# TritonDataCenter/containerpilot

Hardware: NVIDIA H100
Metric: events/sec through Bus.Publish (deliveries/s = 32-byte records landed in subscriber mailboxes) (higher is better)
Workload: dtype u8

## Files before the change

containerpilot_b200/csrc/cpbus.cu:

```cuda
#include "cpbus_kernels.cuh"

#include <algorithm>
#include <chrono>
#include <cstdio>
#include <cstdlib>
#include <cstring>
#include <deque>
#include <mutex>
#include <new>
#include <string>
#include <thread>
#include <unordered_map>
#include <vector>

using namespace cpbus_dev;

namespace {

thread_local char g_cuda_err[256] = "";

#define CK(call)                                                                                   \
  do {                                                                                             \
    cudaError_t e_ = (call);                                                                       \
    if (e_ != cudaSuccess) {                                                                       \
// ... 250 lines not shown
  }
  cudaLaunchConfig_t cfg{};
  cfg.gridDim = dim3(grid); cfg.blockDim = dim3(kThreads); cfg.dynamicSmemBytes = smem; cfg.stream = b->stream;
  cudaLaunchAttribute attr[1];
  attr[0].id = cudaLaunchAttributeProgrammaticStreamSerialization;
  attr[0].val.programmaticStreamSerializationAllowed = 1;
  cfg.attrs = attr; cfg.numAttrs = b->pdl && kind != kLaunchRound ? 1 : 0;
  CK(cudaLaunchKernelEx(&cfg, kernel, p));
  CK(cudaGetLastError());
  return CPBUS_OK;
}

uint64_t max_window(const cpbus* b);

template <int ST>
int preload_round_fanouts() {
  void (*ks[])(FanoutParams) = {
      fanout_round_kernel<ST, false, false, false>, fanout_round_kernel<ST, false, true, false>,
      fanout_round_kernel<ST, true, false, false>, fanout_round_kernel<ST, true, true, false>,
      fanout_round_kernel<ST, false, false, true>, fanout_round_kernel<ST, false, true, true>,
      fanout_round_kernel<ST, true, false, false, true>, fanout_round_kernel<ST, true, true, false, true>};
  for (auto k : ks) CK(cudaFuncSetAttribute(k, cudaFuncAttributeMaxDynamicSharedMemorySize, kFanoutMaxSmem));
  return CPBUS_OK;
}

int preload_round_kernels(cpbus* b) {
  static bool done[64] = {};
  static std::mutex mu;
  std::lock_guard<std::mutex> g(mu);
  if (done[b->device & 63]) return CPBUS_OK;
  int rc;
  if ((rc = preload_round_fanouts<CPBUS_STORE_V4>()) || (rc = preload_round_fanouts<CPBUS_STORE_V8>()) ||
      (rc = preload_round_fanouts<CPBUS_STORE_BULK>()))
    return rc;
  cudaFuncAttributes a;
  CK(cudaFuncGetAttributes(&a, stream_round_decide_kernel));
  CK(cudaFuncGetAttributes(&a, stream_round_admit_kernel));
  CK(cudaFuncGetAttributes(&a, stream_round_agree_kernel));
  CK(cudaFuncGetAttributes(&a, consume_all_kernel));
  CK(cudaFuncGetAttributes(&a, digest_fold_kernel));
  done[b->device & 63] = true;
  return CPBUS_OK;
}

struct StreamArgs {
  const StreamHdr* hdr = nullptr; unsigned long long* ack = nullptr; unsigned long long seq = 0;
  const StreamHdr* next_hdr = nullptr;
  uint32_t off = 0; bool final = true;
  FollowRec* follow_rec = nullptr;
  bool follow_from_host = false;
  const RoundDev* round = nullptr;
};

int launch_fanout(cpbus* b, const cpbus_event* d_src, uint32_t n, uint64_t w, int staged = 0,
                  const cpbus_event* prefetch_src = nullptr, cpbus_event* prefetch_dst = nullptr, uint32_t prefetch_n = 0,
                  bool batch_dep = false, bool account = false, const StreamArgs* sa = nullptr) {
  if (b->n_next == 0 && !sa) return CPBUS_OK;
  if (n == 0 && b->n_timers == 0 && !sa) return CPBUS_OK;
  FanoutParams p{};
  p.batch = d_src; p.ring = b->d_ring; p.ctl = b->d_ctl; p.timers = b->d_timers; p.stats = b->d_stats; p.pow_table = b->d_pow; p.launch_seq = ++b->launch_seq;
  p.desc = b->d_desc + (p.launch_seq & 1) * ((fanout_desc_bytes(2048) + 255) & ~(size_t)255);
  p.desc_ready = b->d_desc_ready + (p.launch_seq & 1) * 16; p.w_now = w;
  p.result = b->d_result + (size_t)(p.launch_seq % kResultRing) * kResultSub;
  p.result_next = b->d_result + (size_t)((p.launch_seq + 1) % kResultRing) * kResultSub;
  p.batch_local = b->d_batch_local; p.staged = (uint32_t)staged;
  p.err_word = b->d_err; p.acct = account ? b->d_acct : nullptr;
  p.pf_state = b->d_pf_state; p.pf_buf = b->d_pf_buf; p.pf_stride = b->B; p.spin_us = b->stream_spin_us;
  if (sa) {
    p.stream_hdr = sa->hdr; p.stream_ack = sa->ack; p.stream_seq = sa->seq; p.stream_next_hdr = sa->next_hdr;
    p.stream_off = sa->off; p.stream_final = sa->final ? 1u : 0u;
  }
  const bool follow = sa && sa->follow_rec, round = sa && sa->round;
  const int kind = round ? kLaunchRound : follow ? kLaunchFollow : kLaunchPlain;
  p.round = round ? sa->round : nullptr;
  if (follow) {
    p.follow_clock = b->d_follow_clock; p.follow_rec = sa->follow_rec; p.follow_window = max_window(b);
    p.follow_from_host = sa->follow_from_host ? 1u : 0u;
  }
  p.prefetch_src = prefetch_src; p.prefetch_dst = prefetch_dst; p.prefetch_n = prefetch_n;
  p.batch_dep = batch_dep ? 1u : 0u; p.n_ev = n;
  p.n_subs = b->n_next; p.ring_cap = b->R; p.K = b->K; p.sub_base = b->cfg.sub_id_base;
  p.use_digest = b->use_digest; p.lossless = b->lossless; p.timers_on = b->n_timers > 0 && b->K > 0;
  p.smem_cap = (n + 31u) & ~31u;
  const size_t hot_bytes = (size_t)b->n_next * (sizeof(SubCtl) + (p.timers_on ? b->K * sizeof(DevTimer) : 0));
  p.hints = b->hints >= 0 ? (uint32_t)b->hints : (hot_bytes <= (64u << 20) ? 1u : 0u);
  const uint32_t need = (b->n_next + kWarpsPerCta - 1) / kWarpsPerCta;
  uint32_t grid = b->cfg.grid_ctas ? std::max(1u, std::min(b->cfg.grid_ctas, need)) : 0u;
  int rc;
  const bool pairs_on = b->n_paired > 0 && b->d_pairs;
  p.pairs = pairs_on ? b->d_pairs : nullptr;
  size_t smem = fanout_smem_bytes(p.smem_cap) + (pairs_on ? kPairFilterBytes : 0);
  if (!pairs_on && !p.timers_on && b->n_filtered > 0) {
    if (b->order_dirty) { const int rc_order = rebuild_order(b); if (rc_order) return rc_order; }
    if (b->n_order) {
      const uint32_t scale = std::max(1u, (p.n_ev + 128u) / 256u);
      uint32_t spw = b->subs_per_warp ? std::min(32u, b->subs_per_warp)
                                      : std::max(4u, std::min(16u / scale, b->n_order / (20480u * scale)));
      p.order = b->d_order; p.n_order = b->n_order; p.spw = spw;
      const uint32_t warps = (b->n_order + spw - 1) / spw;
      grid = std::max(1u, (warps + kWarpsPerCta - 1) / kWarpsPerCta);
    }
  }
  if (pairs_on && !b->cfg.grid_ctas) {
    const uint32_t blocks = (b->n_next + 31u) / 32u;
    grid = std::max(1u, std::min((blocks + kWarpsPerCta - 1) / kWarpsPerCta, (uint32_t)b->sm_count * 16u));
  }
  if (!pairs_on && !p.order) {
    uint32_t spw = b->subs_per_warp;
    if (grid) spw = std::max(1u, (need + grid - 1) / grid);
    else if (!spw) {
      const uint32_t scale = std::max(1u, (p.n_ev + 128u) / 256u);
      const uint32_t cap = std::max(1u, 16u / scale);
      spw = std::max(1u, std::min(cap, (need + (uint32_t)b->sm_count * 7 * scale) / ((uint32_t)b->sm_count * 14 * scale)));
    }
    p.spw = spw;
    grid = std::max(1u, (need + spw - 1) / spw);
    const size_t off = fanout_stage_off(p.smem_cap);
    const size_t per_sub = sizeof(SubCtl) + (p.timers_on ? (size_t)b->K * sizeof(DevTimer) : 0);
    const size_t min_round = (size_t)kWarpsPerCta * per_sub;
    const size_t ctas = std::max<size_t>(1, std::min<size_t>(kCtasPerSm, b->smem_per_sm / (off + min_round + b->smem_reserved)));
    const size_t room = std::min<size_t>(kFanoutMaxSmem, b->smem_per_sm / ctas - b->smem_reserved) - off;
    p.stage_subs = std::max<uint32_t>(kWarpsPerCta, (uint32_t)std::min<size_t>((size_t)kWarpsPerCta * spw, room / per_sub) & ~7u);
    smem = off + p.stage_subs * per_sub;
  }
  const int variant = pairs_on ? (p.use_digest ? 7 : 6) : (p.timers_on ? 2 : 0) | (p.use_digest ? 1 : 0) | (p.order ? 4 : 0);
#define CPBUS_DISPATCH(ST)                                                                \
  switch (variant) {                                                                     \
    case 0: rc = launch_fanout_t<ST, false, false, false>(b, p, grid, smem, kind); break;      \
    case 1: rc = launch_fanout_t<ST, false, true, false>(b, p, grid, smem, kind); break;       \
    case 2: rc = launch_fanout_t<ST, true, false, false>(b, p, grid, smem, kind); break;       \
    case 3: rc = launch_fanout_t<ST, true, true, false>(b, p, grid, smem, kind); break;        \
    case 4: rc = launch_fanout_t<ST, false, false, true>(b, p, grid, smem, kind); break;       \
    case 5: rc = launch_fanout_t<ST, false, true, true>(b, p, grid, smem, kind); break;        \
    case 6: rc = launch_fanout_t<ST, true, false, false, true>(b, p, grid, smem, kind); break; \
    default: rc = launch_fanout_t<ST, true, true, false, true>(b, p, grid, smem, kind); break; \
  }
  switch (b->store) {
    case CPBUS_STORE_V4: CPBUS_DISPATCH(CPBUS_STORE_V4); break;
    case CPBUS_STORE_BULK: CPBUS_DISPATCH(CPBUS_STORE_BULK); break;
    default: CPBUS_DISPATCH(CPBUS_STORE_V8); break;
  }
#undef CPBUS_DISPATCH
  if (rc) return rc;
  b->st.kernel_launches++;
  if (round) return CPBUS_OK;
  b->st.batches++;
  if (follow) return CPBUS_OK;
  b->last_watermark = w;
  if (account && n) dbg_mark_device_batch(b, p.launch_seq);
  return CPBUS_OK;
}

bool admit_fits(cpbus* b, uint32_t n, uint64_t w) {
  if (!b->lossless || b->n_next == 0) return true;
  const uint64_t need = admit_need(n, w, b->last_watermark, b->min_period, b->K, b->n_timers && b->K);
  if (b->room_lb >= need) { b->room_lb -= need; b->st.admit_skipped++; return true; }
  return false;
}

int admit_pass(cpbus* b, const cpbus_event* d_src, uint32_t n, uint64_t w, bool* ok, uint32_t* prefix) {
  CK(cudaMemsetAsync(&b->d_stats->admit_overflow, 0, 4 * sizeof(unsigned long long), b->stream));
  const uint32_t threads = 256, grid = (b->n_next + threads - 1) / threads;
  admit_kernel<<<grid, threads, 0, b->stream>>>(d_src, n, w, b->d_ctl, b->d_timers, b->n_next, b->R, b->K,
                                                b->cfg.sub_id_base, b->n_timers > 0 && b->K > 0, b->d_stats,
                                                b->n_paired > 0 ? b->d_pairs : nullptr);
  CK(cudaGetLastError());
  b->st.kernel_launches++; b->st.admit_passes++;
  CK(cudaMemcpyAsync(&b->h_stats->admit_overflow, &b->d_stats->admit_overflow, 4 * sizeof(unsigned long long),
// ... 1652 lines not shown
```

containerpilot_b200/csrc/cpbus_fanout_body.cuh:

```cuda
  constexpr bool STAGED = !ORDERED && !PAIRS;
  extern __shared__ __align__(128) unsigned char smem[];
  const uint32_t cap = p.smem_cap;
  cpbus_event* s_batch = reinterpret_cast<cpbus_event*>(smem);
  uint64_t* s_rhash = reinterpret_cast<uint64_t*>(smem + (size_t)cap * 32);
  uint2* s_meta = reinterpret_cast<uint2*>(smem + (size_t)cap * 40);
  uint64_t* s_q = reinterpret_cast<uint64_t*>(smem + (size_t)cap * 48);
  uint32_t* s_dsum = reinterpret_cast<uint32_t*>(s_q + cap + 2);
  uint32_t* s_present = s_dsum + 40;
  uint64_t* s_pow = s_q + cap + 2 + 20 + (PAIRS ? kPairFilterWords / 2 : 0);
  BatchSummary* s_sum = reinterpret_cast<BatchSummary*>(s_pow + cap + 66);
  uint32_t* s_tick = reinterpret_cast<uint32_t*>(s_sum + 1);
  const uint4* s_ctl4 = reinterpret_cast<const uint4*>(smem + fanout_stage_off(cap));
  const uint4* s_tim4 = s_ctl4 + 2u * p.stage_subs;

  const int tid = threadIdx.x, lane = tid & 31, warp = tid >> 5;
  uint32_t n = FOLLOW ? 0u : p.n_ev;
  uint64_t w_follow = 0;
  unsigned long long round_ack = 0;

  if (p.batch_dep) asm volatile("griddepcontrol.wait;" ::: "memory");
  const bool stream = p.staged == 2u;
  const uint32_t pf_slot = stream ? (uint32_t)(p.stream_seq % kStreamPrefetch) : 0u;
  uint32_t pos = ORDERED ? (blockIdx.x * kWarpsPerCta + warp) * p.spw : 0u;
  uint32_t my_ids = 0;
  if (ORDERED && pos + lane < min(pos + p.spw, p.n_order)) my_ids = __ldg(p.order + pos + lane);
  if (tid == 0) {
    mbar_init(&s_sum->mbar, 1); mbar_init(&s_sum->mbar_desc, 1); mbar_init(&s_sum->mbar_state, 1);
    s_sum->acc_deliv = 0; s_sum->acc_ticks = 0; s_sum->acc_dig_lo = 0; s_sum->acc_dig_hi = 0;
    s_sum->stream_local = (stream && !p.lossless && p.stream_off == 0 && __ldcg(p.pf_state + pf_slot) == p.stream_seq) ? 1u : 0u;
    s_sum->own_desc = blockIdx.x == 0 ? 1u : 0u; s_sum->abort_launch = 0;
  }
  __syncthreads();
  const bool stream_local = stream && s_sum->stream_local;
  const bool staged = FOLLOW || (p.staged && !stream_local);
  const cpbus_event* batch_src = stream_local ? p.pf_buf + (size_t)pf_slot * p.pf_stride : p.batch;
  if (tid == 0) {
    const uint32_t pow_bytes = ((cap + 65u) * 8u + 15u) & ~15u;
    const bool direct = n && !staged;
    mbar_expect_tx(&s_sum->mbar, (direct ? n * 32u : 0u) + pow_bytes);
    if (direct) bulk_g2s(s_batch, batch_src, n * 32u, &s_sum->mbar);
    bulk_g2s(s_pow, p.pow_table, pow_bytes, &s_sum->mbar);
  }

  const bool keep = p.hints & 1u;

  const uint32_t desc_bytes = 24u * cap + 16u + 160u + (PAIRS ? kPairFilterBytes : 0u);
  uint4* s_desc = reinterpret_cast<uint4*>(s_rhash);
  uint4* g_desc = reinterpret_cast<uint4*>(p.desc);
  constexpr unsigned long long kAbortBit = 1ull << 63;
  if (blockIdx.x != 0) {
    if (tid == 0) {
      unsigned long long seen = 0;
      if (!(p.hints & 2u)) {
        unsigned long long t0, t1;
        asm volatile("mov.u64 %0, %%globaltimer;" : "=l"(t0));
        const unsigned long long budget = stream ? 4000000000ull : 200000ull;
        do {
          asm volatile("ld.acquire.gpu.global.u64 %0, [%1];" : "=l"(seen) : "l"(p.desc_ready) : "memory");
          if ((seen & ~kAbortBit) >= p.launch_seq) break;
          asm volatile("mov.u64 %0, %%globaltimer;" : "=l"(t1));
        } while (t1 - t0 < budget);
      }
      if ((seen & ~kAbortBit) < p.launch_seq) s_sum->own_desc = 1u;
      else {
        const bool ab = (seen & kAbortBit) != 0;
        s_sum->abort_launch = ab ? 1u : 0u;
        asm volatile("fence.proxy.async;" ::: "memory");
        mbar_expect_tx(&s_sum->mbar_desc, desc_bytes);
        bulk_g2s(s_desc, g_desc, desc_bytes, &s_sum->mbar_desc);
        const uint32_t n_copy = FOLLOW ? (ab ? 0u : *reinterpret_cast<const volatile uint32_t*>(p.desc + 24u * cap + 16u + 4u * kFollowN)) : n;
        if (staged && n_copy && !ab) {
          mbar_wait(&s_sum->mbar, 0);
          mbar_expect_tx(&s_sum->mbar, n_copy * 32u);
          bulk_g2s(s_batch, p.batch_local, n_copy * 32u, &s_sum->mbar);
        }
      }
    }
    __syncthreads();
  }
  const bool own_desc = s_sum->own_desc != 0;
  const bool lead = blockIdx.x == 0;
  if (own_desc) {
    if (lead && tid < kResultSub * 4) reinterpret_cast<unsigned long long*>(p.result_next)[tid] = 0ull;
    if (tid < 40) s_dsum[tid] = 0;
    if constexpr (ROUND) {
      __syncthreads();
      if (tid == 0) {
        const volatile RoundDev* rd = p.round;
        if (!rd->go) s_sum->abort_launch = 1u;
        else {
          const unsigned long long w = rd->w;
          s_dsum[kFollowN] = rd->m; s_dsum[kFollowWLo] = (uint32_t)w; s_dsum[kFollowWHi] = (uint32_t)(w >> 32);
          s_dsum[kRoundSrc] = rd->src;
          if (lead && rd->final) round_ack = rd->q;
        }
      }
    } else if constexpr (FOLLOW) {
      __syncthreads();
      if (tid == 0) {
        unsigned long long seen = 0, t0, t1, tag = 0, prev = p.w_now, hw = 0;
        const unsigned long long budget = (p.spin_us ? (unsigned long long)p.spin_us : 2000000ull) * 1000ull;
        asm volatile("mov.u64 %0, %%globaltimer;" : "=l"(t0));
        unsigned int err = 0;
        uint32_t hn = 0;
        if (!p.follow_from_host) {
          const unsigned long long* pw = p.follow_clock + 2u * (uint32_t)((p.launch_seq - 1ull) & 1ull);
          for (;;) {
            asm volatile("ld.acquire.gpu.global.u64 %0, [%1];" : "=l"(tag) : "l"(pw + 1) : "memory");
            if (tag == p.launch_seq - 1ull) break;
            asm volatile("mov.u64 %0, %%globaltimer;" : "=l"(t1));
            if (t1 - t0 > budget) break;
            __nanosleep(64);
          }
          if (tag != p.launch_seq - 1ull) err = kErrStreamTimeout;
          else asm volatile("ld.relaxed.gpu.global.u64 %0, [%1];" : "=l"(prev) : "l"(pw) : "memory");
        }
        const bool skip = !err && prev == kFollowPoison;
        if (!err && !skip) {
          for (;;) {
            asm volatile("ld.acquire.sys.global.u64 %0, [%1];" : "=l"(seen) : "l"(&p.stream_hdr->seq) : "memory");
            if (seen >= p.stream_seq) break;
            asm volatile("mov.u64 %0, %%globaltimer;" : "=l"(t1));
            if (t1 - t0 > budget) break;
            __nanosleep(64);
          }
          if (seen != p.stream_seq) err = kErrStreamTimeout;
          else {
// ... 85 lines not shown
      const uint32_t lo = min(nd, (uint32_t)tid * E), hi = min(nd, lo + E);
      uint64_t sum = 0;
      for (uint32_t i = lo; i < hi; i++) sum += s_rhash[i] * s_pow[nd - 1 - i];
      uint64_t incl = sum;
#pragma unroll
      for (int o = 1; o < 32; o <<= 1) {
        const uint32_t l = __shfl_up_sync(0xffffffffu, (uint32_t)incl, o), h = __shfl_up_sync(0xffffffffu, (uint32_t)(incl >> 32), o);
        if (lane >= o) incl += ((uint64_t)h << 32) | l;
      }
      if (lane == 31) s_sum->red[warp] = incl;
      __syncthreads();
      uint64_t run = incl - sum;
      for (int w = 0; w < warp; w++) run += s_sum->red[w];
      for (uint32_t i = lo; i < hi; i++) { s_q[i] = run; run += s_rhash[i] * s_pow[nd - 1 - i]; }
      if (tid == 0) { uint64_t t = 0; for (int w = 0; w < kWarpsPerCta; w++) t += s_sum->red[w]; s_q[nd] = t; }
      __syncthreads();
    }
    if (PAIRS) {
      for (uint32_t i = tid; i < kPairFilterWords; i += kThreads) s_present[i] = 0u;
      __syncthreads();
      for (uint32_t i = tid; i < nd; i += kThreads) {
        if (s_meta[i].y != CPBUS_TARGET_ALL) continue;
        const uint32_t h = pair_key_hash(s_batch[i].code, s_batch[i].source_id);
        atomicOr(&s_present[(h & 32767u) >> 5], 1u << (h & 31u));
        atomicOr(&s_present[((h >> 15) & 32767u) >> 5], 1u << ((h >> 15) & 31u));
      }
      __syncthreads();
    }
    if (lead) {
      for (uint32_t i = tid; i < desc_bytes / 16u; i += kThreads) g_desc[i] = s_desc[i];
      __threadfence();
      __syncthreads();
      if (tid == 0) {
        const unsigned long long flag = p.launch_seq | (ab ? kAbortBit : 0ull);
        asm volatile("st.release.gpu.global.u64 [%0], %1;" ::"l"(p.desc_ready), "l"(flag) : "memory");
      }
    }
  } else {
    mbar_wait(&s_sum->mbar_desc, 0);
    if constexpr (FOLLOW) {
      n = s_sum->abort_launch ? 0u : s_dsum[kFollowN];
      w_follow = ((uint64_t)s_dsum[kFollowWHi] << 32) | s_dsum[kFollowWLo];
    }
    mbar_wait(&s_sum->mbar, (staged && n && !s_sum->abort_launch) ? 1u : 0u);
  }
  constexpr bool PLANAR = STORE != CPBUS_STORE_BULK && !ORDERED;
  const uint32_t hi_off = cap;
  if (PLANAR && n) {
    uint4* sq = reinterpret_cast<uint4*>(s_batch);
    uint4 v[8];
    __syncthreads();
#pragma unroll
    for (int r = 0; r < 8; r++) { const uint32_t q = tid + r * kThreads; if (q < 2u * n) v[r] = sq[q]; }
    __syncthreads();
#pragma unroll
    for (int r = 0; r < 8; r++) { const uint32_t q = tid + r * kThreads; if (q < 2u * n) sq[(q & 1u) * hi_off + (q >> 1)] = v[r]; }
    __syncthreads();
  }
  auto ev_ts = [&](uint32_t i) -> uint64_t {
    return PLANAR ? reinterpret_cast<const uint64_t*>(reinterpret_cast<const uint4*>(s_batch) + i)[1] : s_batch[i].ts_ns;
  };
  auto ev_code_src = [&](uint32_t i) -> uint2 {
    return PLANAR ? reinterpret_cast<const uint2*>(reinterpret_cast<const uint4*>(s_batch) + hi_off + i)[0] : make_uint2(s_batch[i].code, s_batch[i].source_id);
  };
  const bool aborted = s_sum->abort_launch != 0;
  const uint32_t K = p.K, J = K ? 32u / K : 32u;
  const uint32_t tk_slot = lane / J, tk_j = lane % J;
  const bool timers_on = TIMERS && p.timers_on && K;
  const uint32_t wstride = gridDim.x * kWarpsPerCta;
  uint32_t pos_end = (aborted || !ORDERED) ? 0u : min(pos + p.spw, p.n_order);
  const uint32_t pos_step = ORDERED ? 1u : kWarpsPerCta;
  const uint32_t pos0 = pos;
  uint32_t s = ORDERED ? __shfl_sync(0xffffffffu, my_ids, 0) : pos;
  if (!p.batch_dep) asm volatile("griddepcontrol.wait;" ::: "memory");
  asm volatile("griddepcontrol.launch_dependents;");
  const uint32_t rng_first = blockIdx.x * kWarpsPerCta * p.spw, rng_end = min(rng_first + kWarpsPerCta * p.spw, p.n_subs);
  auto stage_round = [&](uint32_t first) {
    if (!STAGED || tid != 0 || aborted || first >= rng_end) return;
    const uint32_t rn = min(p.stage_subs, rng_end - first);
    asm volatile("fence.proxy.async.shared::cta;" ::: "memory");
    const uint32_t tim_bytes = timers_on ? rn * K * (uint32_t)sizeof(DevTimer) : 0u;
    mbar_expect_tx(&s_sum->mbar_state, rn * (uint32_t)sizeof(SubCtl) + tim_bytes);
    bulk_g2s_hint(const_cast<uint4*>(s_ctl4), p.ctl + first, rn * (uint32_t)sizeof(SubCtl), &s_sum->mbar_state, keep);
    if (tim_bytes) bulk_g2s_hint(const_cast<uint4*>(s_tim4), p.timers + (size_t)first * K, tim_bytes, &s_sum->mbar_state, keep);
  };
  uint4 ca = make_uint4(0, 0, 0, 0), cb = ca, ta = ca;
  if (ORDERED && pos < pos_end) ld_sector(p.ctl + s, ca, cb, keep);
  const uint32_t present = s_dsum[0];
  const bool has_unicast = s_dsum[1] != 0;
  bool bulk_pending = false;
  uint32_t tri_blk = blockIdx.x * kWarpsPerCta + warp, tri_base = 0, tri_live = 0;
  uint4 tri_a = make_uint4(0, 0, 0, 0), tri_b = tri_a;
  uint32_t rnd_first = rng_first, rnd_phase = 0;
  for (;;) {
  if constexpr (STAGED) {
    if (aborted || rnd_first >= rng_end) break;
    stage_round(rnd_first);
    mbar_wait(&s_sum->mbar_state, rnd_phase);
    rnd_phase ^= 1u;
    pos = rnd_first + warp; pos_end = rnd_first + min(p.stage_subs, rng_end - rnd_first);
  }
  if constexpr (PAIRS) {
    bool exhausted = aborted;
    while (!tri_live && !exhausted) {
      tri_base = tri_blk * 32u;
      if (tri_base >= p.n_subs) { exhausted = true; break; }
      tri_blk += wstride;
      const uint32_t sl = tri_base + lane;
      bool live = false;
      tri_a = make_uint4(0, 0, 0, 0); tri_b = tri_a;
      if (sl < p.n_subs) ld_sector(p.ctl + sl, tri_a, tri_b, keep);
      const uint32_t ml = tri_b.z;
      if (ml & kActiveBit) {
        live = has_unicast || (ml & present) != 0;
        if (!live && timers_on) {
          const uint32_t nsl = min((ml >> kTimerHintShift) & 0xFu, K);
          for (uint32_t t = 0; t < nsl && !live; t++) {
            uint4 h;
            ld_half(p.timers + (size_t)sl * K + t, h, keep);
            const uint64_t due = ((uint64_t)h.y << 32) | h.x;
            live = due != kTimerIdle && due <= (FOLLOW ? w_follow : p.w_now);
          }
        }
        if (!live && (ml & kPairBit)) {
          const uint4* row = reinterpret_cast<const uint4*>(p.pairs + (size_t)sl * CPBUS_MAX_PAIRS);
          for (uint32_t q = 0; q < CPBUS_MAX_PAIRS / 2 && !live; q++) {
            const uint4 v = __ldg(row + q);
            if (v.x >= 32u) break;
            uint32_t h = pair_key_hash(v.x, v.y);
            live = ((s_present[(h & 32767u) >> 5] >> (h & 31u)) & (s_present[((h >> 15) & 32767u) >> 5] >> ((h >> 15) & 31u)) & 1u) != 0;
            if (live || v.z >= 32u) { if (!live) break; continue; }
            h = pair_key_hash(v.z, v.w);
            live = ((s_present[(h & 32767u) >> 5] >> (h & 31u)) & (s_present[((h >> 15) & 32767u) >> 5] >> ((h >> 15) & 31u)) & 1u) != 0;
          }
        }
      }
      tri_live = __ballot_sync(0xffffffffu, live);
    }
    if (exhausted) break;
    const uint32_t jl = (uint32_t)__ffs(tri_live) - 1u;
    tri_live &= tri_live - 1u;
    pos = tri_base + jl; pos_end = pos + 1u; s = pos;
    ca = make_uint4(__shfl_sync(0xffffffffu, tri_a.x, jl), __shfl_sync(0xffffffffu, tri_a.y, jl), __shfl_sync(0xffffffffu, tri_a.z, jl), __shfl_sync(0xffffffffu, tri_a.w, jl));
    cb = make_uint4(__shfl_sync(0xffffffffu, tri_b.x, jl), __shfl_sync(0xffffffffu, tri_b.y, jl), __shfl_sync(0xffffffffu, tri_b.z, jl), __shfl_sync(0xffffffffu, tri_b.w, jl));
    if (timers_on && tk_slot < K) ld_half(p.timers + (size_t)s * K + tk_slot, ta, keep);
  }
  const uint32_t Rm = p.ring_cap - 1;
  const uint4* s4 = reinterpret_cast<const uint4*>(s_batch);
  const uint32_t scratch_words = max(32u, cap / 2u);
  uint32_t* my_tick = s_tick + warp * scratch_words;

  uint32_t run_mask = 0xffffffffu, run_k = 0;
  uint64_t run_sum = 0;
  for (; pos < pos_end; pos += pos_step) {
    const uint32_t si = pos - rnd_first;
    uint4 cur_a = ca, cur_b = cb;
    auto ctl_half = [&](uint32_t h) -> uint4 { return STAGED ? s_ctl4[2u * si + h] : (h ? cur_b : cur_a); };
    auto tim_half = [&](uint32_t h) -> uint4 {
      if (STAGED) return s_tim4[2u * (si * K + tk_slot) + h];
      if (!h) return ta;
      uint4 cold;
      ld_half(reinterpret_cast<const unsigned char*>(p.timers + (size_t)s * K + tk_slot) + 16, cold, keep);
      return cold;
    };
    if (STAGED) { cur_a = ctl_half(0); cur_b = ctl_half(1); }
    if (ORDERED) s = __shfl_sync(0xffffffffu, my_ids, (pos - pos0) & 31); else s = pos;
    if (ORDERED) {
      const uint32_t pn = pos + pos_step;
      if (pn < pos_end) ld_sector(p.ctl + __shfl_sync(0xffffffffu, my_ids, (pn - pos0) & 31), ca, cb, keep);
    }
    const uint32_t m = cur_b.z;
    if (!(m & kActiveBit)) continue;
    const uint64_t tail = ((uint64_t)cur_a.y << 32) | cur_a.x;
    cpbus_event* ring = p.ring + (size_t)s * p.ring_cap;
    const uint32_t gid = p.sub_base + s;
    const uint32_t nslots = timers_on ? min((m >> kTimerHintShift) & 0xFu, K) : 0u;
    const bool dense = !has_unicast && ((m & present) == present);

    uint32_t n_ticks = 0, tk_mask = 0, tk_rank = 0, tk_src = 0, tk_fired = 0;
    bool tk_valid = false; uint64_t tk_due = 0, tk_period = 0;
    if (nslots) {
      uint64_t tk_due0 = kTimerIdle;
      if (TIMERS && tk_slot < nslots) {
        const uint4 hot = tim_half(0);
        tk_due0 = ((uint64_t)hot.y << 32) | hot.x; tk_period = ((uint64_t)hot.w << 32) | hot.z;
      }
      tk_due = tk_due0 + (uint64_t)tk_j * tk_period;
      tk_valid = tk_due0 != kTimerIdle && tk_due <= (FOLLOW ? w_follow : p.w_now) && (tk_j == 0 || tk_period != 0);
      tk_mask = __ballot_sync(0xffffffffu, tk_valid);
      n_ticks = __popc(tk_mask);
      if (n_ticks) {

        if (J == 32 || (tk_mask >> J) == 0) tk_rank = tk_j;
        else {
#pragma unroll 1
          for (int t = 0; t < 32; t++) {
            if (!((tk_mask >> t) & 1u)) continue;
            const uint64_t od = shfl64(tk_due, t);
            const uint32_t os = __shfl_sync(0xffffffffu, tk_slot, t);
            tk_rank += (od < tk_due || (od == tk_due && os < tk_slot)) ? 1u : 0u;
          }
        }
      }
    }
    uint32_t tk_pos = 0;
    if (tk_valid) {
      uint32_t lo = 0, hi = n;
      while (lo < hi) {
        const uint32_t mid = (lo + hi) >> 1;
        if (ev_ts(mid) < tk_due) lo = mid + 1; else hi = mid;
      }
      tk_pos = lo;
    }

    bool pair_live = false;
    if (PAIRS && (m & kPairBit) && !dense) {
      uint2 pr = make_uint2(kPairNone, 0u);
      if (lane < CPBUS_MAX_PAIRS) pr = __ldg(p.pairs + (size_t)s * CPBUS_MAX_PAIRS + lane);
      bool hit = false;
      if (pr.x < 32u) {
        const uint32_t h = pair_key_hash(pr.x, pr.y);
        hit = ((s_present[(h & 32767u) >> 5] >> (h & 31u)) & (s_present[((h >> 15) & 32767u) >> 5] >> ((h >> 15) & 31u)) & 1u) != 0;
      }
      pair_live = __any_sync(0xffffffffu, hit);
    }
    if (PAIRS && !pair_live && !has_unicast && n_ticks == 0 && (m & present) == 0) continue;

    uint32_t k = 0;
    uint64_t dsum = 0;

    if (dense && n_ticks == 0) {
      if (STORE == CPBUS_STORE_BULK) {
        if (lane == 0 && n) {
          const uint32_t slot0 = (uint32_t)tail & Rm;
          const uint32_t first = min(n, p.ring_cap - slot0);
          bulk_s2g(ring + slot0, s_batch, first * 32u);
          if (n > first) bulk_s2g(ring, s_batch + first, (n - first) * 32u);
          asm volatile("cp.async.bulk.commit_group;" ::: "memory");
        }
        bulk_pending = true;
      } else if (STORE == CPBUS_STORE_V8) {
        for (uint32_t c0 = 0; c0 < n; c0 += 32)
          copy_record_pairs<PLANAR>(s4, hi_off, ring, (uint32_t)tail, Rm, c0 + lane, c0 + lane, c0 + lane < n);
      } else {
        for (uint32_t q = lane; q < 2 * n; q += 32) {
          const uint4 v = PLANAR ? s4[(q & 1u) * hi_off + (q >> 1)] : s4[q];
          st_v4(reinterpret_cast<unsigned char*>(ring + (((uint32_t)tail + (q >> 1)) & Rm)) + (q & 1u) * 16u, v);
        }
      }
      k = n;
      if (DIGEST) dsum = s_q[n];
    } else if (dense) {
      constexpr bool cold_early = !STAGED;
      if (cold_early && TIMERS && tk_slot < nslots) {
        const uint4 cold = tim_half(1);
        tk_src = cold.x; tk_fired = cold.y;
      }
      if (tk_valid) my_tick[tk_rank] = tk_pos;
      __syncwarp();
      k = n + n_ticks;
      const uint32_t T = (uint32_t)lane < n_ticks ? my_tick[lane] : 0xFFFFFFFFu;
      auto slot_of = [&](uint32_t c0) -> uint32_t {
        const uint32_t before = __popc(__ballot_sync(0xffffffffu, T <= c0));
        const bool in = T > c0 && T < c0 + 32u;
        const uint32_t n_in = __popc(__ballot_sync(0xffffffffu, in));
        const uint32_t i = c0 + lane;
        uint32_t out = i + before;
        if (n_in) {
          const uint32_t bits = __reduce_or_sync(0xffffffffu, in ? 1u << (T - c0) : 0u);
          if (__popc(bits) == n_in) out += __popc(bits & ((2u << lane) - 1u));
          else
            for (uint32_t t = before; t < n_ticks && my_tick[t] < c0 + 32u; t++) out += (my_tick[t] <= i) ? 1u : 0u;
        }
        return out;
      };
      uint32_t c0 = 0;
#pragma unroll 1
      for (; c0 + 64 <= n; c0 += 64) {
        const uint32_t o0 = slot_of(c0), o1 = slot_of(c0 + 32);
        copy_record_pairs<PLANAR>(s4, hi_off, ring, (uint32_t)tail, Rm, c0 + lane, o0, true);
        copy_record_pairs<PLANAR>(s4, hi_off, ring, (uint32_t)tail, Rm, c0 + 32 + lane, o1, true);
      }
#pragma unroll 1
      for (; c0 < n; c0 += 32) {
        const uint32_t out = slot_of(c0);
        copy_record_pairs<PLANAR>(s4, hi_off, ring, (uint32_t)tail, Rm, c0 + lane, out, c0 + lane < n);
      }
      if (!cold_early && TIMERS && tk_slot < nslots) {
        const uint4 cold = tim_half(1);
        tk_src = cold.x; tk_fired = cold.y;
      }
      if (tk_valid) {
        const uint32_t out = tk_pos + tk_rank;
        const uint64_t w0 = (uint64_t)tk_fired + tk_j, w1 = tk_due;
        const uint64_t w2 = (uint64_t)CPBUS_TIMER_EXPIRED | ((uint64_t)tk_src << 32);
        const uint64_t w3 = (uint64_t)gid | ((uint64_t)CPBUS_F_TICK << 32);
        const uint4 a = make_uint4((uint32_t)w0, (uint32_t)(w0 >> 32), (uint32_t)w1, (uint32_t)(w1 >> 32));
        const uint4 b = make_uint4((uint32_t)w2, (uint32_t)(w2 >> 32), (uint32_t)w3, (uint32_t)(w3 >> 32));
        st_v8(ring + (((uint32_t)tail + out) & Rm), a, b);
        if (DIGEST) {
          const uint32_t prev = tk_rank ? my_tick[tk_rank - 1] : 0u;
          dsum = (s_q[tk_pos] - s_q[prev]) * s_pow[n_ticks - tk_rank] + record_hash_words(w0, w1, w2, w3) * s_pow[k - 1 - out];
          if (tk_rank == n_ticks - 1) dsum += s_q[n] - s_q[tk_pos];
        }
      }
      if (DIGEST) dsum = warp_sum64(dsum);
      __syncwarp();
    } else if (!(PAIRS && pair_live) && !has_unicast && n_ticks == 0) {
      if constexpr (!TIMERS) {
        uint16_t* my_idx = reinterpret_cast<uint16_t*>(my_tick);
        const bool reuse = ORDERED && (m & CPBUS_MASK_ALL) == run_mask;
        if (!reuse) {
          uint32_t base = 0;
          const uint32_t nchunks = (n + 31) >> 5;
          for (uint32_t c0 = 0; c0 < nchunks; c0 += 4) {
            uint32_t cbit[4];
#pragma unroll
            for (uint32_t u = 0; u < 4; u++) {
              const uint32_t i = (c0 + u) * 32 + lane;
              cbit[u] = i < n ? s_meta[i].x : 0u;
            }
#pragma unroll
            for (uint32_t u = 0; u < 4; u++) {
              const bool match = (m & cbit[u]) != 0;
              const uint32_t w = __ballot_sync(0xffffffffu, match);
              if (match) my_idx[base + __popc(w & ((1u << lane) - 1u))] = (uint16_t)((c0 + u) * 32 + lane);
              base += __popc(w);
            }
          }
          run_k = base;
          __syncwarp();
        }
        k = run_k;
        uint64_t acc = 0;
// ... 49 lines not shown
        const bool used = my_pair.x < 32u;
        n_pairs = __popc(__ballot_sync(0xffffffffu, used));
        pair_codes = __reduce_or_sync(0xffffffffu, used ? (1u << my_pair.x) : 0u);
      }
      uint32_t myword = 0;
      for (uint32_t c = 0; c < nchunks; c++) {
        const uint32_t i = c * 32 + lane;
        bool match = false, cand = false;
        if (i < n) {
          const uint2 mt = s_meta[i];
          match = (mt.y == CPBUS_TARGET_ALL) ? ((m & mt.x) != 0) : (mt.y == gid);
          if (PAIRS) cand = !match && mt.y == CPBUS_TARGET_ALL && (mt.x & pair_codes) != 0;
        }
        if (PAIRS && n_pairs && __any_sync(0xffffffffu, cand)) {
          uint32_t ev_code = kPairNone - 1u, ev_src = 0;
          if (cand) { const uint2 cs = ev_code_src(i); ev_code = cs.x; ev_src = cs.y; }
          for (uint32_t j = 0; j < n_pairs; j++) {
            const uint32_t pc = __shfl_sync(0xffffffffu, my_pair.x, j), ps = __shfl_sync(0xffffffffu, my_pair.y, j);
            match = match || (ev_code == pc && ev_src == ps);
          }
        }
        const uint32_t w = __ballot_sync(0xffffffffu, match);
        if ((uint32_t)lane == c) myword = w;
      }
      uint32_t wcount = __popc(myword), wprefix = wcount;
#pragma unroll
      for (int o = 1; o < 32; o <<= 1) {
        const uint32_t t = __shfl_up_sync(0xffffffffu, wprefix, o);
        if (lane >= o) wprefix += t;
      }
      const uint32_t k_ev = __shfl_sync(0xffffffffu, wprefix, 31);
      wprefix -= wcount;
      uint32_t tk_mp = 0;
      if (n_ticks) {
        const uint32_t pc = tk_pos >> 5;
        const uint32_t wsel = __shfl_sync(0xffffffffu, myword, pc & 31);
        const uint32_t psel = __shfl_sync(0xffffffffu, wprefix, pc & 31);
        tk_mp = (tk_pos >= n) ? k_ev : psel + __popc(wsel & ((1u << (tk_pos & 31u)) - 1u));
        if (tk_valid) my_tick[tk_rank] = tk_mp;
        __syncwarp();
      }
      k = k_ev + n_ticks;
      for (uint32_t c = 0; c < nchunks; c++) {
        const uint32_t w = __shfl_sync(0xffffffffu, myword, c);
        const uint32_t wp = __shfl_sync(0xffffffffu, wprefix, c);
        if (!w) continue;
        const bool mine = (w >> lane) & 1u;
        const uint32_t i = c * 32 + lane;
        uint32_t out = 0;
        if (mine) {
          const uint32_t mrank = wp + __popc(w & ((1u << lane) - 1u));
          out = mrank;
          for (uint32_t t = 0; t < n_ticks; t++) out += (my_tick[t] <= mrank) ? 1u : 0u;
          if (DIGEST) dsum += s_rhash[i] * s_pow[k - 1 - out];
        }
        copy_record_pairs<PLANAR>(s4, hi_off, ring, (uint32_t)tail, Rm, i, out, mine);
      }
      if (n_ticks) {
        if (TIMERS && tk_slot < nslots) {
          const uint4 cold = tim_half(1);
          tk_src = cold.x; tk_fired = cold.y;
        }
      }
      if (tk_valid) {
        const uint32_t out = tk_mp + tk_rank;
        const uint64_t w0 = (uint64_t)tk_fired + tk_j, w1 = tk_due;
        const uint64_t w2 = (uint64_t)CPBUS_TIMER_EXPIRED | ((uint64_t)tk_src << 32);
        const uint64_t w3 = (uint64_t)gid | ((uint64_t)CPBUS_F_TICK << 32);
        const uint4 a = make_uint4((uint32_t)w0, (uint32_t)(w0 >> 32), (uint32_t)w1, (uint32_t)(w1 >> 32));
        const uint4 b = make_uint4((uint32_t)w2, (uint32_t)(w2 >> 32), (uint32_t)w3, (uint32_t)(w3 >> 32));
        st_v8(ring + (((uint32_t)tail + out) & Rm), a, b);
        if (DIGEST) dsum += record_hash_words(w0, w1, w2, w3) * s_pow[k - 1 - out];
      }
      if (DIGEST) dsum = warp_sum64(dsum);
      __syncwarp();
    }

    if (n_ticks) {
      const uint32_t slotmask = (J == 32 ? 0xffffffffu : ((1u << J) - 1u)) << (tk_slot * J);
      const uint32_t fired_here = __popc(tk_mask & slotmask);
      if (TIMERS && tk_j == 0 && tk_slot < nslots && fired_here) {
        unsigned char* t = reinterpret_cast<unsigned char*>(&p.timers[(size_t)s * K + tk_slot]);
        const uint64_t nd = tk_period ? tk_due + (uint64_t)fired_here * tk_period : kTimerIdle;
        st_half(t, make_uint4((uint32_t)nd, (uint32_t)(nd >> 32), (uint32_t)tk_period, (uint32_t)(tk_period >> 32)), keep);
        st_half(t + 16, make_uint4(tk_src, tk_fired + fired_here, 0u, 0u), keep);
      }
    }
    if (lane == 0 && k) {
      const uint4 c0 = ctl_half(0), c1 = ctl_half(1);
      const uint64_t dig = ((uint64_t)c1.y << 32) | c1.x;
      const uint64_t nt = tail + k;
      const uint64_t nd = DIGEST ? dig * s_pow[k] + dsum : dig;
      st_sector(p.ctl + s, make_uint4((uint32_t)nt, (uint32_t)(nt >> 32), c0.z, c0.w),
                make_uint4((uint32_t)nd, (uint32_t)(nd >> 32), m, 0u), keep);
      atomicAdd(&s_sum->acc_deliv, k);
      if (DIGEST) {
        const uint32_t f = (uint32_t)nd ^ (uint32_t)(nd >> 32);
        atomicAdd(&s_sum->acc_dig_lo, f & 0xFFFFu);
        atomicAdd(&s_sum->acc_dig_hi, f >> 16);
      }
      if (TIMERS && n_ticks) atomicAdd(&s_sum->acc_ticks, n_ticks);
    }
  }

  if constexpr (ORDERED) break;
  if constexpr (STAGED) {
    __syncthreads();
    rnd_first += p.stage_subs;
  }
  }
  if (STORE == CPBUS_STORE_BULK && bulk_pending && lane == 0)
    asm volatile("cp.async.bulk.wait_group 0;" ::: "memory");
  __syncthreads();
  if (tid == 0) {
    DevStatSlot* st = &p.stats->slot[blockIdx.x % kStatSlots];
    if (s_sum->acc_deliv) atomicAdd(&st->deliveries, (unsigned long long)s_sum->acc_deliv);
    if (s_sum->acc_ticks) atomicAdd(&st->ticks, (unsigned long long)s_sum->acc_ticks);
    DevResultSlot* rs = &p.result[blockIdx.x % kResultSub];
    if (s_sum->acc_deliv) atomicAdd(&rs->deliveries, (unsigned long long)s_sum->acc_deliv);
    if (s_sum->acc_ticks) atomicAdd(&rs->ticks, (unsigned long long)s_sum->acc_ticks);
    if (s_sum->acc_dig_lo | s_sum->acc_dig_hi) atomicAdd(&rs->digest_sum, (unsigned long long)s_sum->acc_dig_lo + ((unsigned long long)s_sum->acc_dig_hi << 16));
    if (blockIdx.x == 0) atomicAdd(&rs->launch_seq, p.launch_seq);
  }
  if (blockIdx.x == 0 && p.acct && !aborted) {
    if (tid < 32 && tid != CPBUS_METRIC && s_dsum[2 + tid]) atomicAdd(&p.acct->by_code[tid], (unsigned long long)s_dsum[2 + tid]);
    for (uint32_t i = tid; i < n; i += kThreads) {
      if (s_meta[i].y != CPBUS_TARGET_ALL) continue;
      const uint2 cs = ev_code_src(i);
      const uint32_t code = cs.x;
      if (code == CPBUS_METRIC || code >= 32u) continue;
      const unsigned long long key = (((unsigned long long)code << 32) | cs.y) + 1ull;
      uint32_t slot = pair_key_hash(code, cs.y) & (kAcctPairSlots - 1u);
      bool placed = false;
      for (int probe = 0; probe < 32 && !placed; probe++, slot = (slot + 1u) & (kAcctPairSlots - 1u)) {
        const unsigned long long old = atomicCAS(&p.acct->pair_key[slot], 0ull, key);
        if (old == 0ull || old == key) { atomicAdd(&p.acct->pair_cnt[slot], 1ull); placed = true; }
      }
      if (!placed) atomicAdd(&p.acct->pair_overflow, 1ull);
    }
    if (tid == 0) {
      DevDbgTail* t = &p.acct->tail[p.launch_seq % kAcctDbgRing];
      uint32_t* idx = s_tick;
      uint32_t kept = 0, nb = 0;
      for (uint32_t c = 0; c < 32; c++) nb += s_dsum[2 + c];
      for (uint32_t i = n; i > 0 && kept < (uint32_t)kAcctDbgKeep; i--)
        if (s_meta[i - 1].y == CPBUS_TARGET_ALL) idx[kept++] = i - 1;
      for (uint32_t j = 0; j < kept; j++) {
        const uint32_t i = idx[kept - 1 - j];
        if (PLANAR) {
          uint4* o = reinterpret_cast<uint4*>(&t->ev[j]);
          o[0] = reinterpret_cast<const uint4*>(s_batch)[i]; o[1] = reinterpret_cast<const uint4*>(s_batch)[hi_off + i];
        } else t->ev[j] = s_batch[i];
      }
      t->n_broadcast = nb; t->n_kept = kept;
      __threadfence();
      t->launch_seq = p.launch_seq;
    }
  }
  if (blockIdx.x == 0 && p.prefetch_src) {
    uint32_t pn = p.prefetch_n;
    bool go = true;
    if (stream) {
      if (tid == 0) {
        unsigned long long seen; uint32_t hn = 0;
        asm volatile("ld.acquire.sys.global.u64 %0, [%1];" : "=l"(seen) : "l"(&p.stream_next_hdr->seq) : "memory");
        bool ok = !aborted && seen == p.stream_seq + 2;
        if (ok) {
          asm volatile("ld.relaxed.sys.global.u32 %0, [%1];" : "=r"(hn) : "l"(&p.stream_next_hdr->n) : "memory");
// ... 24 lines not shown
```

containerpilot_b200/csrc/cpbus_kernels.cuh:

```cuda
#pragma once
#include <cstdint>
#include <cuda_runtime.h>

#include "../../include/cpbus.h"

namespace cpbus_dev {

constexpr int kWarpsPerCta = 8;
constexpr int kThreads = kWarpsPerCta * 32;
constexpr int kCtasPerSm = 4;
constexpr uint32_t kActiveBit = 0x80000000u;
constexpr int kTimerHintShift = 24;
constexpr uint32_t kPairBit = 0x10000000u;
constexpr uint32_t kPairNone = 0xFFFFFFFFu;
constexpr uint32_t kPairFilterWords = 1024;
constexpr uint32_t kPairFilterBytes = kPairFilterWords * 4;
__host__ __device__ inline uint32_t pair_key_hash(uint32_t code, uint32_t source_id) {
  uint32_t x = (source_id ^ (code << 27)) * 0x9E3779B1u;
  x ^= x >> 15; x *= 0x85EBCA77u; x ^= x >> 13;
  return x;
}
constexpr uint64_t kDigestP = 0x9E3779B97F4A7C15ull;
constexpr uint32_t kPowTableLen = 2048 + 65 + 7;

struct __align__(32) DevTimer {
  uint64_t next_due;
  uint64_t period;
  uint32_t source_id;
  uint32_t fired;
  uint32_t pad[2];
};
constexpr uint64_t kTimerIdle = ~0ull;

constexpr int kStatSlots = 256;
struct __align__(32) DevStatSlot { unsigned long long deliveries, ticks, pad[2]; };
struct DevStats {
  DevStatSlot slot[kStatSlots];
  unsigned long long admit_overflow, overwritten;
  unsigned long long admit_max_used;
  unsigned long long admit_deficit;
};

constexpr uint32_t kAcctPairSlots = 1u << 19;
constexpr int kAcctDbgRing = 64, kAcctDbgKeep = 10;
struct __align__(32) DevDbgTail {
  unsigned long long launch_seq;
  uint32_t n_broadcast, n_kept;
  cpbus_event ev[kAcctDbgKeep];
  uint32_t pad[4];
};
struct DevPubAcct {
  unsigned long long by_code[32];
  unsigned long long pair_overflow, pad[3];
  DevDbgTail tail[kAcctDbgRing];
  unsigned long long pair_key[kAcctPairSlots];
  unsigned long long pair_cnt[kAcctPairSlots];
};

struct __align__(32) SubCtl {
  unsigned long long tail;
  unsigned long long head;
  unsigned long long digest;
  uint32_t mask;
  uint32_t pad;
};

constexpr int kResultRing = 64, kResultSub = 8;
struct __align__(32) DevResultSlot { unsigned long long deliveries, ticks, digest_sum, launch_seq; };

struct __align__(32) StreamHdr { unsigned long long seq, watermark; uint32_t n, pad[3]; };
struct __align__(32) StreamMeta { uint32_t magic, n_slots, batch_cap, n_consumers, pad[4]; };
constexpr uint32_t kStreamMagic = 0x53425043u;
constexpr uint32_t kStreamMaxConsumers = 64;
constexpr int kStreamPrefetch = 3;
constexpr unsigned int kErrStreamTimeout = 1u, kErrStreamShape = 2u;
constexpr unsigned int kErrFollowOrder = 4u;
constexpr unsigned long long kFollowPoison = ~0ull;
enum : uint32_t { kFollowDelivered = 0u, kFollowAborted = 1u, kFollowSkipped = 2u, kFollowPending = 0xFFFFFFFFu };
struct __align__(16) FollowRec { uint32_t n, status; unsigned long long watermark; };
constexpr uint32_t kFollowN = 34, kFollowWLo = 35, kFollowWHi = 36;
__host__ __device__ inline size_t stream_hdr_off() { return sizeof(StreamMeta); }
__host__ __device__ inline size_t stream_ack_off(uint32_t n_slots) { return stream_hdr_off() + (size_t)n_slots * sizeof(StreamHdr); }
__host__ __device__ inline size_t stream_payload_off(uint32_t n_slots) { return stream_ack_off(n_slots) + (size_t)kStreamMaxConsumers * 32; }
__host__ __device__ inline size_t stream_bytes(uint32_t n_slots, uint32_t batch_cap) { return stream_payload_off(n_slots) + (size_t)n_slots * batch_cap * 32; }

constexpr unsigned long long kOfferRoundMask = (1ull << 31) - 1;
__host__ __device__ inline uint32_t stream_offer_word_index(uint32_t consumer, unsigned long long round) {
  return 4u * consumer + 1u + (uint32_t)(round & 1ull);
}
__host__ __device__ inline unsigned long long stream_offer_word(unsigned long long round, uint32_t stalled, uint32_t prefix) {
  return ((round & kOfferRoundMask) << 33) | ((unsigned long long)(stalled ? 1u : 0u) << 32) | prefix;
}
struct __align__(16) StreamAgreeResult { uint32_t m, stalled, status, pad; };

__host__ __device__ inline uint64_t admit_need(uint64_t n, uint64_t w, uint64_t last_wm, uint64_t min_period, uint32_t K,
                                              bool timers_armed) {
  if (!timers_armed) return n;
  const uint64_t per_slot = (min_period != ~0ull && w > last_wm) ? (w - last_wm) / min_period + 2 : 2;
  return n + (uint64_t)K * per_slot;
}

struct __align__(16) RoundCursor { unsigned long long batch; uint32_t off, pad; };
enum : uint32_t { kRoundOk = 0u, kRoundSkip = 1u, kRoundAbort = 2u };
enum : uint32_t { kRoundAdmitNone = 0u, kRoundAdmitSkipped = 1u, kRoundAdmitPass = 2u };
struct __align__(32) RoundDev {
  unsigned long long room;
  unsigned long long now, last_wm;
  unsigned long long poison;
  unsigned long long room_full;
  unsigned long long q, hw;
  uint32_t off, rem, status, admit;
  unsigned long long w;
  uint32_t go, m, src, final;
};
enum : uint32_t { kRoundPartial = 3u, kRoundStalled = 4u };
// ... 665 lines not shown
```

Before: 92.75 billion.

## Tier L2 persistence hints for timers and add interleaved dense tick-merge path

Splits the L2 keep hint so that when control plus timer state fits a 64MB budget but not 32MB, only subscriber control blocks get the evict-last hint and timer loads and stores use normal policy. It also adds a dense-path variant for non-pair launches where each warp writes batch events and expired-timer tick records interleaved in 16-byte halves, computing tick positions with ballots and reductions, and computes the digest in closed form from prefix sums. The goal is to keep hot control data resident in L2 and to merge ticks into the event stream without a separate serial pass. The risks are extra shuffle and ballot work per chunk and a more complex digest calculation that must match the old ordering exactly.

```diff
diff --git a/containerpilot_b200/csrc/cpbus.cu b/containerpilot_b200/csrc/cpbus.cu
--- a/containerpilot_b200/csrc/cpbus.cu
+++ b/containerpilot_b200/csrc/cpbus.cu
@@ -356,8 +356,10 @@
   p.n_subs = b->n_next; p.ring_cap = b->R; p.K = b->K; p.sub_base = b->cfg.sub_id_base;
   p.use_digest = b->use_digest; p.lossless = b->lossless; p.timers_on = b->n_timers > 0 && b->K > 0;
   p.smem_cap = (n + 31u) & ~31u;
-  const size_t hot_bytes = (size_t)b->n_next * (sizeof(SubCtl) + (p.timers_on ? b->K * sizeof(DevTimer) : 0));
-  p.hints = b->hints >= 0 ? (uint32_t)b->hints : (hot_bytes <= (64u << 20) ? 1u : 0u);
+  const size_t ctl_bytes = (size_t)b->n_next * sizeof(SubCtl);
+  const size_t hot_bytes = ctl_bytes + (p.timers_on ? (size_t)b->n_next * b->K * sizeof(DevTimer) : 0);
+  p.hints = b->hints >= 0 ? (uint32_t)b->hints
+                          : hot_bytes <= (32u << 20) ? 1u : hot_bytes <= (64u << 20) ? 1u | kHintNoTimers : 0u;
   const uint32_t need = (b->n_next + kWarpsPerCta - 1) / kWarpsPerCta;
   uint32_t grid = b->cfg.grid_ctas ? std::max(1u, std::min(b->cfg.grid_ctas, need)) : 0u;
   int rc;
diff --git a/containerpilot_b200/csrc/cpbus_fanout_body.cuh b/containerpilot_b200/csrc/cpbus_fanout_body.cuh
--- a/containerpilot_b200/csrc/cpbus_fanout_body.cuh
+++ b/containerpilot_b200/csrc/cpbus_fanout_body.cuh
@@ -43,6 +43,7 @@
   }
 
   const bool keep = p.hints & 1u;
+  const bool keep_tim = keep && !(p.hints & kHintNoTimers);
 
   const uint32_t desc_bytes = 24u * cap + 16u + 160u + (PAIRS ? kPairFilterBytes : 0u);
   uint4* s_desc = reinterpret_cast<uint4*>(s_rhash);
@@ -294,7 +295,7 @@
     const uint32_t tim_bytes = timers_on ? rn * K * (uint32_t)sizeof(DevTimer) : 0u;
     mbar_expect_tx(&s_sum->mbar_state, rn * (uint32_t)sizeof(SubCtl) + tim_bytes);
     bulk_g2s_hint(const_cast<uint4*>(s_ctl4), p.ctl + first, rn * (uint32_t)sizeof(SubCtl), &s_sum->mbar_state, keep);
-    if (tim_bytes) bulk_g2s_hint(const_cast<uint4*>(s_tim4), p.timers + (size_t)first * K, tim_bytes, &s_sum->mbar_state, keep);
+    if (tim_bytes) bulk_g2s_hint(const_cast<uint4*>(s_tim4), p.timers + (size_t)first * K, tim_bytes, &s_sum->mbar_state, keep_tim);
   };
   uint4 ca = make_uint4(0, 0, 0, 0), cb = ca, ta = ca;
   if (ORDERED && pos < pos_end) ld_sector(p.ctl + s, ca, cb, keep);
@@ -329,7 +330,7 @@
           const uint32_t nsl = min((ml >> kTimerHintShift) & 0xFu, K);
           for (uint32_t t = 0; t < nsl && !live; t++) {
             uint4 h;
-            ld_half(p.timers + (size_t)sl * K + t, h, keep);
+            ld_half(p.timers + (size_t)sl * K + t, h, keep_tim);
             const uint64_t due = ((uint64_t)h.y << 32) | h.x;
             live = due != kTimerIdle && due <= (FOLLOW ? w_follow : p.w_now);
           }
@@ -355,7 +356,7 @@
     pos = tri_base + jl; pos_end = pos + 1u; s = pos;
     ca = make_uint4(__shfl_sync(0xffffffffu, tri_a.x, jl), __shfl_sync(0xffffffffu, tri_a.y, jl), __shfl_sync(0xffffffffu, tri_a.z, jl), __shfl_sync(0xffffffffu, tri_a.w, jl));
     cb = make_uint4(__shfl_sync(0xffffffffu, tri_b.x, jl), __shfl_sync(0xffffffffu, tri_b.y, jl), __shfl_sync(0xffffffffu, tri_b.z, jl), __shfl_sync(0xffffffffu, tri_b.w, jl));
-    if (timers_on && tk_slot < K) ld_half(p.timers + (size_t)s * K + tk_slot, ta, keep);
+    if (timers_on && tk_slot < K) ld_half(p.timers + (size_t)s * K + tk_slot, ta, keep_tim);
   }
   const uint32_t Rm = p.ring_cap - 1;
   const uint4* s4 = reinterpret_cast<const uint4*>(s_batch);
@@ -372,7 +373,7 @@
       if (STAGED) return s_tim4[2u * (si * K + tk_slot) + h];
       if (!h) return ta;
       uint4 cold;
-      ld_half(reinterpret_cast<const unsigned char*>(p.timers + (size_t)s * K + tk_slot) + 16, cold, keep);
+      ld_half(reinterpret_cast<const unsigned char*>(p.timers + (size_t)s * K + tk_slot) + 16, cold, keep_tim);
       return cold;
     };
     if (STAGED) { cur_a = ctl_half(0); cur_b = ctl_half(1); }
@@ -462,6 +463,65 @@
       }
       k = n;
       if (DIGEST) dsum = s_q[n];
+    } else if (dense && !PAIRS) {
+      if (TIMERS && tk_slot < nslots) {
+        const uint4 cold = tim_half(1);
+        tk_src = cold.x; tk_fired = cold.y;
+      }
+      if (tk_valid) my_tick[tk_rank] = tk_pos | ((uint32_t)lane << 16);
+      __syncwarp();
+      k = n + n_ticks;
+      const uint32_t a = (uint32_t)tail & 15u, end = a + k;
+      uint32_t Pk = 0x00FFFFFFu;
+      if ((uint32_t)lane < n_ticks) { const uint32_t t = my_tick[lane]; Pk = ((t >> 16) << 24) | ((t & 0xFFFFu) + lane + a); }
+      const uint32_t h = lane & 1u, d = (uint32_t)lane >> 1;
+      constexpr uint32_t G = 2;
+#pragma unroll 1
+      for (uint32_t u0 = 0; u0 < end; u0 += 16u * G) {
+        const uint32_t Pa = Pk & 0x00FFFFFFu;
+        const uint32_t before = __popc(__ballot_sync(0xffffffffu, Pa < u0));
+        const uint32_t bits = __reduce_or_sync(0xffffffffu, Pa - u0 < 16u * G ? 1u << (Pa - u0) : 0u);
+        uint4 v[G];
+        uint32_t rk[G];
+        bool tk[G];
+#pragma unroll
+        for (uint32_t g = 0; g < G; g++) {
+          const uint32_t off = 16u * g + d, u = u0 + off;
+          tk[g] = (bits >> off) & 1u;
+          rk[g] = before + __popc(bits & ((1u << off) - 1u));
+          const uint32_t e = (u >= a && u < end && !tk[g]) ? u - a - rk[g] : 0u;
+          v[g] = PLANAR ? s4[h * hi_off + e] : s4[2u * e + h];
+        }
+        if (bits) {
+#pragma unroll
+          for (uint32_t g = 0; g < G; g++) {
+            const uint32_t sl = __shfl_sync(0xffffffffu, Pk, tk[g] ? rk[g] : 0u) >> 24;
+            const uint64_t q = shfl64((uint64_t)tk_fired + tk_j, sl), du = shfl64(tk_due, sl);
+            const uint32_t sr = __shfl_sync(0xffffffffu, tk_src, sl);
+            if (tk[g]) v[g] = h ? make_uint4(CPBUS_TIMER_EXPIRED, sr, gid, CPBUS_F_TICK)
+                                : make_uint4((uint32_t)q, (uint32_t)(q >> 32), (uint32_t)du, (uint32_t)(du >> 32));
+          }
+        }
+#pragma unroll
+        for (uint32_t g = 0; g < G; g++) {
+          const uint32_t u = u0 + 16u * g + d;
+          if (u >= a && u < end) st_v4(reinterpret_cast<unsigned char*>(ring + (((uint32_t)tail - a + u) & Rm)) + 16u * h, v[g]);
+        }
+      }
+      if (DIGEST) {
+        const uint32_t t = (uint32_t)lane < n_ticks ? my_tick[lane] : 0u, T = t & 0xFFFFu, sl = t >> 16;
+        const uint64_t r_seq = shfl64((uint64_t)tk_fired + tk_j, sl), r_due = shfl64(tk_due, sl);
+        const uint32_t r_src = __shfl_sync(0xffffffffu, tk_src, sl);
+        if ((uint32_t)lane < n_ticks) {
+          const uint32_t prev = lane ? (my_tick[lane - 1] & 0xFFFFu) : 0u;
+          const uint64_t w2 = (uint64_t)CPBUS_TIMER_EXPIRED | ((uint64_t)r_src << 32);
+          const uint64_t w3 = (uint64_t)gid | ((uint64_t)CPBUS_F_TICK << 32);
+          dsum = (s_q[T] - s_q[prev]) * s_pow[n_ticks - lane] + record_hash_words(r_seq, r_due, w2, w3) * s_pow[k - 1 - (T + lane)];
+          if ((uint32_t)lane == n_ticks - 1) dsum += s_q[n] - s_q[T];
+        }
+      }
+      if (DIGEST) dsum = warp_sum64(dsum);
+      __syncwarp();
     } else if (dense) {
       constexpr bool cold_early = !STAGED;
       if (cold_early && TIMERS && tk_slot < nslots) {
@@ -677,8 +737,8 @@
       if (TIMERS && tk_j == 0 && tk_slot < nslots && fired_here) {
         unsigned char* t = reinterpret_cast<unsigned char*>(&p.timers[(size_t)s * K + tk_slot]);
         const uint64_t nd = tk_period ? tk_due + (uint64_t)fired_here * tk_period : kTimerIdle;
-        st_half(t, make_uint4((uint32_t)nd, (uint32_t)(nd >> 32), (uint32_t)tk_period, (uint32_t)(tk_period >> 32)), keep);
-        st_half(t + 16, make_uint4(tk_src, tk_fired + fired_here, 0u, 0u), keep);
+        st_half(t, make_uint4((uint32_t)nd, (uint32_t)(nd >> 32), (uint32_t)tk_period, (uint32_t)(tk_period >> 32)), keep_tim);
+        st_half(t + 16, make_uint4(tk_src, tk_fired + fired_here, 0u, 0u), keep_tim);
       }
     }
     if (lane == 0 && k) {
diff --git a/containerpilot_b200/csrc/cpbus_kernels.cuh b/containerpilot_b200/csrc/cpbus_kernels.cuh
--- a/containerpilot_b200/csrc/cpbus_kernels.cuh
+++ b/containerpilot_b200/csrc/cpbus_kernels.cuh
@@ -31,6 +31,7 @@
   uint32_t pad[2];
 };
 constexpr uint64_t kTimerIdle = ~0ull;
+constexpr uint32_t kHintNoTimers = 4u;
 
 constexpr int kStatSlots = 256;
 struct __align__(32) DevStatSlot { unsigned long long deliveries, ticks, pad[2]; };
```

Measured after the change: 94.53 billion, median of 6. 1.9% higher.
